# confluentinc/quickstart-streaming-agents

Measured on AMD Instinct MI355X. Metric: lab1_price_match_agent_decisions_per_sec, higher is better.
Workload: dtype bf16; 1 GPU; model=llama3-8b, global_batch=192, seq_len=2048, agent_loop=model_driven_grammar, parallelism=dp1

## Files before the change

quickstart_streaming_agents_amd/models/llama.py:

```python

from __future__ import annotations

import os
from dataclasses import dataclass

import torch
import torch.nn.functional as F

from ..ops import dispatch as D
from .kv_cache import PagedKVCache

PREFILL_V1 = os.environ.get("QSA_PREFILL_V1") == "1"
DECODE_V1 = os.environ.get("QSA_DECODE_V1") == "1"
PREFILL_TILE_ROWS = 32


@dataclass
class LlamaConfig:
    name: str = "llama3-8b"
    vocab_size: int = 128_256
    hidden: int = 4096
    n_layers: int = 32
    n_q_heads: int = 32
    n_kv_heads: int = 8
# ... 123 lines not shown
                if want(self.lm_head.shape):
                    self.lm_head_f = D.pack_weight_frag(self.lm_head)

    def _ffn_weights(self, w, rows, cols) -> dict:
        c = self.cfg
        wgu_full = w(2 * c.ffn, c.hidden)
        wgu = torch.cat([rows(wgu_full[:c.ffn], self.tp_size),
                         rows(wgu_full[c.ffn:], self.tp_size)],
                        dim=0).contiguous()
        wdown = cols(w(c.hidden, c.ffn, std=0.02 / (2 * c.n_layers) ** 0.5),
                     self.tp_size)
        return {"wgu": wgu, "wdown": wdown}

    def new_kv_cache(self, n_pages: int) -> PagedKVCache:
        return PagedKVCache(self.cfg.n_layers, self.n_kv, self.cfg.d_head,
                            n_pages, self.device, self.dtype)

    def _linear(self, x: torch.Tensor, w: torch.Tensor,
                wf: torch.Tensor | None = None,
                wf8: tuple | None = None) -> torch.Tensor:
        n, k = w.shape
        M = x.shape[0]
        if x.is_cuda and wf8 is not None:
            if M <= 32:
                return D.skinny_linear_fp8(x, wf8[0], wf8[1], n, k)
            import os as _os
            if _os.environ.get("QSA_FP8_BATCH") == "1" and M <= 256 \
                    and n % 64 == 0 and n <= 32768:
                wgs = n // 64
                splitk = 1 if wgs >= 256 else (2 if wgs >= 128 else 4)
                if k % (64 * splitk) == 0:
                    return D.gemm_fp8_batch(x, wf8[0], wf8[1], n, k,
                                            splitk)
        if x.is_cuda and M <= 32 and wf is not None and \
                n * k <= 6144 * 4096:
            return D.skinny_linear(x, wf, n, k)
        return F.linear(x, w)

    def _tp_all_reduce(self, t: torch.Tensor) -> torch.Tensor:
        if self.tp_size > 1:
            import torch.distributed as dist
            dist.all_reduce(t, group=self.tp_group)
        return t

    def _split_qkv(self, qkv: torch.Tensor, n: int):
        c = self.cfg
        qd = self.n_q * c.d_head
# ... 216 lines not shown
```

quickstart_streaming_agents_amd/models/serve.py:

```python

from __future__ import annotations

import time
from dataclasses import dataclass, field

import torch

from .llama import LlamaModel


@dataclass
class Sequence:
    seq_id: int
    prompt: list[int]
    max_new_tokens: int
    cached_len: int = 0
    out_tokens: list[int] = field(default_factory=list)
    done: bool = False
    keep_alive: bool = False
    decision_allowed: list[int] | None = None
    branches: dict[int, list[int]] | None = None
    script: list[int] | None = None


@dataclass
class EngineStats:
    prefill_tokens: int = 0
    cached_prefix_tokens: int = 0
    decode_tokens: int = 0
    decode_steps: int = 0
    jump_forward_tokens: int = 0
    prefills: int = 0
    prefill_batches: int = 0
    wall_s: float = 0.0
    prefill_s: float = 0.0
    decode_s: float = 0.0


import os as _os
_TIMING = _os.environ.get("QSA_TIMING", "") == "1"
_TUNABLE_DONE = False


def _enable_tunableop() -> None:
    global _TUNABLE_DONE
    if _TUNABLE_DONE or _os.environ.get("QSA_NO_TUNABLEOP") == "1":
        return
    _TUNABLE_DONE = True
    try:
        path = _os.path.join(_os.path.dirname(_os.path.abspath(__file__)),
                             "..", "data", "tunableop_mi355x.csv")
        if _os.path.exists(path):
            t = torch.cuda.tunable
            t.enable(True)
            t.tuning_enable(False)
            t.read_file(path)
    except Exception:
        pass


class Engine:
    def __init__(self, model: LlamaModel, kv_pages: int | None = None,
                 max_batch: int = 256, max_seq_len: int = 4096,
                 eos_id: int | None = None, prefill_batch_tokens: int = 65536,
# ... 2 lines not shown
                 decision_temperature: float = 1.0):
        if torch.cuda.is_available():
            _enable_tunableop()
        self.model = model
        self.temperature = float(temperature)
        self.decision_temperature = float(decision_temperature)
        self.jump_forward = _os.environ.get(
            "QSA_NO_JUMP_FORWARD", "") != "1"
        self.max_batch = max_batch
        self.max_seq_len = max_seq_len
        self.eos_id = eos_id
        self.prefill_batch_tokens = prefill_batch_tokens
        if kv_pages is None:
            kv_pages = max_batch * ((max_seq_len + 63) // 64) + 64
        self.kv = model.new_kv_cache(kv_pages)
        self._next_id = 0
        self.pending: list[Sequence] = []
        self.running: list[Sequence] = []
        self.finished: list[Sequence] = []
        self.stats = EngineStats()
        self.use_graph = torch.cuda.is_available() and \
            torch.device(model.device).type == "cuda"
        self._graph = None
        self._graph_failed = False
        self._gbuf: dict = {}
        self._vocab_bias: torch.Tensor | None = None
        if valid_vocab is not None:
            lo, hi = valid_vocab
            bias = torch.full((model.cfg.vocab_size,), float("-inf"),
                              device=model.device, dtype=torch.float32)
            bias[lo:hi] = 0.0
            if self.eos_id is not None:
                bias[self.eos_id] = 0.0
            self._vocab_bias = bias

    def _sample(self, logits: torch.Tensor) -> torch.Tensor:
        if self._vocab_bias is not None:
            logits = logits.float() + self._vocab_bias
        if self.temperature <= 0.0:
            return torch.argmax(logits, dim=-1)
        u = torch.rand(logits.shape, device=logits.device,
                       dtype=torch.float32).clamp_min_(1e-20)
        gumbel = -torch.log(-torch.log(u).clamp_min_(1e-20))
        return torch.argmax(logits.float() + self.temperature * gumbel,
                            dim=-1)

    def _sample_first(self, logits: torch.Tensor,
                      admitted: list["Sequence"]) -> list[int]:
        free = self._sample(logits)
        rows = [i for i, s in enumerate(admitted) if s.decision_allowed]
        if not rows:
# ... 13 lines not shown
            u = torch.rand(sub.shape, device=sub.device).clamp_min_(1e-20)
            sub = sub / t + (-torch.log(-torch.log(u)))
        sub = sub.masked_fill(pad, float("-inf"))
        pick = idx.gather(1, torch.argmax(sub, 1, keepdim=True)).squeeze(1)
        out = free.tolist()
        for r, t in zip(rows, pick.tolist()):
            out[r] = int(t)
        return [int(t) for t in out]

    MAX_RUN = 512

    def _ensure_graph(self) -> bool:
        if self._graph is not None:
            return True
        if self._graph_failed:
            return False
        try:
            self._capture_graph()
            return True
        except Exception:
            self._graph_failed = True
            self.use_graph = False
            self._graph = None
            torch.cuda.synchronize()
            return False

    def _capture_graph(self) -> None:
        dev = self.model.device
        B = self.max_batch
        cap = (self.max_seq_len + 63) // 64
        gb = {
            "tokens": torch.zeros(B, dtype=torch.int64, device=dev),
            "block_table": torch.zeros(B, cap, dtype=torch.int32, device=dev),
            "seq_lens": torch.zeros(B, dtype=torch.int32, device=dev),
            "active": torch.zeros(B, dtype=torch.int32, device=dev),
            "ctr": torch.zeros(1, dtype=torch.int64, device=dev),
            "hist": torch.zeros(self.MAX_RUN, B, dtype=torch.int64, device=dev),
            "script": torch.zeros(B, self.MAX_RUN, dtype=torch.int64,
                                  device=dev),
            "script_mask": torch.zeros(B, self.MAX_RUN, dtype=torch.bool,
                                       device=dev),
        }

        def body():
            gb["seq_lens"].add_(gb["active"])
            positions = (gb["seq_lens"] - 1).clamp(min=0).int()
            logits = self.model.forward_decode(
                gb["tokens"], self.kv, gb["block_table"], gb["seq_lens"],
                positions)
            nxt = self._sample(logits)
            j = gb["ctr"].clamp(max=self.MAX_RUN - 1)
            forced = gb["script"].index_select(1, j).squeeze(1)
            fmask = gb["script_mask"].index_select(1, j).squeeze(1)
            nxt = torch.where(fmask, forced, nxt)
            gb["hist"].index_copy_(0, gb["ctr"], nxt.unsqueeze(0))
            gb["ctr"].add_(1)
            gb["tokens"].copy_(nxt)

        for _ in range(2):
            body()
        gb["ctr"].zero_()
        gb["seq_lens"].zero_()
        torch.cuda.synchronize()
        g = torch.cuda.CUDAGraph()
        with torch.cuda.graph(g):
            body()
        self._graph = g
        self._gbuf = gb

    def _decode_run_eager(self, batch: list[Sequence], run: int) -> None:
        for _ in range(run):
            live = [s for s in batch if not s.done]
            if not live:
                break
            for s in live:
                self.kv.extend(s.seq_id, len(s.prompt) + len(s.out_tokens))
            self._decode_step_eager(live)

    def _decode_step_eager(self, batch: list[Sequence]) -> None:
        dev = self.model.device
        tokens = torch.tensor([s.out_tokens[-1] for s in batch],
                              dtype=torch.int64, device=dev)
        positions = torch.tensor(
            [len(s.prompt) + len(s.out_tokens) - 1 for s in batch],
            dtype=torch.int32, device=dev)
        seq_ids = [s.seq_id for s in batch]
        bt = self.kv.block_table(seq_ids)
        sl = self.kv.seq_lens_tensor(seq_ids)
        logits = self.model.forward_decode(tokens, self.kv, bt, sl,
                                           positions)
        nxt = self._sample(logits).tolist()
        for s, tok in zip(batch, nxt):
            if s.script:
                si = len(s.out_tokens) - 1
                if si < len(s.script):
                    tok = s.script[si]
            s.out_tokens.append(int(tok))
            self._maybe_finish(s)
        self.stats.decode_tokens += len(batch)
        self.stats.decode_steps += 1

    def _decode_run_graph(self, batch: list[Sequence], run: int) -> None:
        if not self._ensure_graph():
            self._decode_run_eager(batch, run)
            return
        self._graph_run_begin(batch, run)
        self._graph_run_end(batch, run)

    def _graph_run_begin(self, batch: list[Sequence], run: int) -> None:
        gb = self._gbuf
        n = len(batch)
        dev = self.model.device
        for s in batch:
            self.kv.extend(s.seq_id, len(s.prompt) + len(s.out_tokens) + run)
            self.kv._seq_len[s.seq_id] = \
                len(s.prompt) + len(s.out_tokens) - 1
        seq_ids = [s.seq_id for s in batch]
        bt = self.kv.block_table(seq_ids)
        gb["block_table"][:n, :bt.shape[1]] = bt
        gb["seq_lens"][:n] = self.kv.seq_lens_tensor(seq_ids)
        gb["tokens"][:n] = torch.tensor([s.out_tokens[-1] for s in batch],
                                        dtype=torch.int64, device=dev)
        gb["active"][:n] = 1
# ... 3 lines not shown
        if any(s.script for s in batch):
            sc = torch.zeros(n, run, dtype=torch.int64)
            sm = torch.zeros(n, run, dtype=torch.bool)
            for i, s in enumerate(batch):
                if not s.script:
                    continue
                d = len(s.out_tokens)
                window = s.script[d - 1: d - 1 + run]
                if window:
                    sc[i, :len(window)] = torch.tensor(window,
                                                       dtype=torch.int64)
                    sm[i, :len(window)] = True
            gb["script"][:n, :run] = sc.to(dev)
            gb["script_mask"][:n, :run] = sm.to(dev)
            gb["script_mask"][:n, run:] = False
            if n < self.max_batch:
                gb["script_mask"][n:] = False
        else:
            gb["script_mask"].fill_(False)
        gb["ctr"].zero_()
        if _TIMING:
            torch.cuda.synchronize()
            self._t_graph0 = time.perf_counter()
        for _ in range(run):
            self._graph.replay()

    def _graph_run_end(self, batch: list[Sequence], run: int) -> None:
        gb = self._gbuf
        n = len(batch)
        if _TIMING:
            torch.cuda.synchronize()
            self.stats.decode_s += time.perf_counter() - self._t_graph0
        hist = gb["hist"][:run, :n].t().tolist()
        for s, toks in zip(batch, hist):
            new = [int(t) for t in toks]
            if self.eos_id is not None and self.eos_id in new:
                new = new[: new.index(self.eos_id) + 1]
            s.out_tokens.extend(new)
            self.kv._seq_len[s.seq_id] = len(s.prompt) + len(s.out_tokens)
            self._maybe_finish(s)
        self.stats.decode_tokens += n * run
        self.stats.decode_steps += run

    def submit(self, prompt_tokens: list[int], max_new_tokens: int,
               continue_from: Sequence | None = None,
               keep_alive: bool = False, constraint=None) -> Sequence:
        prompt = list(prompt_tokens[: self.max_seq_len - 1])
        decision_allowed = branches = None
        if constraint is not None:
            decision_allowed = list(constraint.decision_allowed)
            branches = dict(constraint.branches)
            max_new_tokens = max(max_new_tokens,
                                 constraint.max_script_len() + 1)
            max_new_tokens = min(max_new_tokens, self.MAX_RUN)
        max_new_tokens = max(1, min(max_new_tokens,
                                    self.max_seq_len - len(prompt)))
        if continue_from is not None and not continue_from.keep_alive:
            continue_from = None
        if continue_from is not None:
            shared = min(len(continue_from.prompt), len(prompt) - 1)
            if prompt[:shared] != continue_from.prompt[:shared]:
                shared = 0
            if shared > 0:
                seq = Sequence(continue_from.seq_id, prompt, max_new_tokens,
                               cached_len=shared, keep_alive=keep_alive,
# ... 232 lines not shown
```

quickstart_streaming_agents_amd/ops/dispatch.py:

```python

from __future__ import annotations

import torch

from . import ext


def _cuda(t: torch.Tensor) -> bool:
    return t.is_cuda



def rmsnorm(x: torch.Tensor, w: torch.Tensor, eps: float) -> torch.Tensor:
    if _cuda(x):
        return ext().rmsnorm(x, w, eps)
    xf = x.float()
    y = xf * torch.rsqrt(xf.pow(2).mean(-1, keepdim=True) + eps) * w.float()
    return y.to(x.dtype)


def rmsnorm_residual(x: torch.Tensor, res: torch.Tensor, w: torch.Tensor,
                     eps: float) -> torch.Tensor:
    if _cuda(x):
        return ext().rmsnorm_residual(x, res, w, eps)
# ... 175 lines not shown
                      k: int) -> torch.Tensor:
    q = qf.reshape(n // 16, k // 64, 16, 4, 2, 8) \
        .permute(0, 2, 1, 4, 3, 5).reshape(n, k)
    return q.view(torch.float8_e4m3fn).float() * scale[:, None].float()


def gemm_fp8_batch(x: torch.Tensor, qf: torch.Tensor,
                   scale: torch.Tensor, n: int, k: int,
                   splitk: int = 1) -> torch.Tensor:
    if x.is_cuda:
        return ext().gemm_fp8_batch(x, qf, scale, n, k, splitk)
    w = unpack_weight_fp8(qf, scale, n, k)
    return (x.float() @ w.T).to(x.dtype)


def skinny_linear_fp8(x: torch.Tensor, qf: torch.Tensor,
                      scale: torch.Tensor, n: int, k: int) -> torch.Tensor:
    if x.is_cuda:
        return ext().skinny_gemm_fp8(x, qf, scale, n, k)
    w = unpack_weight_fp8(qf, scale, n, k)
    return (x.float() @ w.T).to(x.dtype)



def topk_cosine(queries: torch.Tensor, docs: torch.Tensor, k: int):
    if _cuda(queries):
        return ext().topk_cosine(queries, docs, k)
    from .cpu_ref import topk_cosine_ref
    return topk_cosine_ref(queries, docs, k)


def window_agg(ts: torch.Tensor, key: torch.Tensor,
               value: torch.Tensor | None, t0: int, win_ms: int, nwin: int,
               nkeys: int):
    if _cuda(ts):
        return ext().window_agg(ts, key, value, t0, win_ms, nwin, nkeys)
    from .cpu_ref import window_agg_ref
    return window_agg_ref(ts, key, value, t0, win_ms, nwin, nkeys)



def hash_build(keys: torch.Tensor, ts: torch.Tensor):
    ts = ts.clamp(min=0, max=(1 << 40) - 1)
    if _cuda(keys):
        return tuple(ext().hash_build(keys, ts.contiguous()))
    table: dict = {}
# ... 17 lines not shown
```

quickstart_streaming_agents_amd/ops/hip/elementwise.hip:

```cpp
#include "common.h"

__global__ void __launch_bounds__(256)
qsa_rmsnorm_kernel(const unsigned short* __restrict__ x,
                   const unsigned short* __restrict__ w,
                   unsigned short* __restrict__ y,
                   unsigned short* __restrict__ res,
                   int H, float eps) {
  const long long row = blockIdx.x;
  const unsigned short* xr = x + row * H;
  unsigned short* yr = y + row * H;
  unsigned short* rr = res ? res + row * H : nullptr;
  __shared__ float scratch[8];

  uint4 buf[4];
  float ss = 0.f;
#pragma unroll
  for (int c = 0; c < 4; ++c) {
    const int i = (threadIdx.x + c * blockDim.x) * 8;
    if (i >= H) break;
    uint4 v = *reinterpret_cast<const uint4*>(xr + i);
    float acc = 0.f;
    unsigned int pk[4] = {v.x, v.y, v.z, v.w};
    if (rr) {
      uint4 rv = *reinterpret_cast<const uint4*>(rr + i);
// ... 273 lines not shown
    uint4 o4;
    unsigned int* oo = reinterpret_cast<unsigned int*>(&o4);
#pragma unroll
    for (int j = 0; j < 4; ++j) {
      float2 f = bf16x2_to_f32x2(vv[j]);
      const float a = (i + 2 * j < limit) ? __expf(f.x * scale - mx) * inv
                                          : 0.f;
      const float b = (i + 2 * j + 1 < limit)
                          ? __expf(f.y * scale - mx) * inv : 0.f;
      oo[j] = f32x2_to_bf16x2(a, b);
    }
    *reinterpret_cast<uint4*>(r + i) = o4;
  }
}

extern "C" void qsa_softmax_rows_bf16_launch(unsigned short* scores,
                                             long long rows, int cols,
                                             float scale,
                                             const int* row_limits,
                                             hipStream_t stream) {
  hipLaunchKernelGGL(qsa_softmax_rows_bf16_kernel, dim3((unsigned)rows),
                     dim3(256), 0, stream, scores, cols, scale, row_limits);
}
```

quickstart_streaming_agents_amd/ops/hip/ops.cpp:

```cpp
#include <hip/hip_runtime.h>
#include <torch/extension.h>
#include <ATen/hip/HIPContext.h>

#define CHK(x) TORCH_CHECK(x, #x)
#define CHK_DEV(t) TORCH_CHECK((t).is_cuda(), #t " must be on the GPU")
#define CHK_CONT(t) TORCH_CHECK((t).is_contiguous(), #t " must be contiguous")
#define CHK_BF16(t) TORCH_CHECK((t).scalar_type() == at::kBFloat16, #t " must be bf16")
#define CHK_F32(t) TORCH_CHECK((t).scalar_type() == at::kFloat, #t " must be f32")
#define CHK_I32(t) TORCH_CHECK((t).scalar_type() == at::kInt, #t " must be i32")

static inline const unsigned short* u16(const torch::Tensor& t) {
  return reinterpret_cast<const unsigned short*>(t.data_ptr());
}
static inline unsigned short* u16m(torch::Tensor& t) {
  return reinterpret_cast<unsigned short*>(t.data_ptr());
}
static inline hipStream_t cur_stream() {
  return at::hip::getCurrentHIPStream().stream();
}

extern "C" void qsa_rmsnorm_launch(const unsigned short*, const unsigned short*,
                                   unsigned short*, unsigned short*, long long,
                                   int, float, hipStream_t);
extern "C" void qsa_swiglu_launch(const unsigned short*, const unsigned short*,
// ... 44 lines not shown
                                          hipStream_t);
extern "C" void qsa_kv_scatter_launch(const unsigned short*,
                                      const unsigned short*, unsigned short*,
                                      unsigned short*, const int*, int, int,
                                      int, long long, hipStream_t);
extern "C" void qsa_skinny_gemm_launch(const unsigned short*,
                                       const unsigned short*, unsigned short*,
                                       int, int, long long, long long,
                                       hipStream_t);
extern "C" void qsa_skinny_gemm_probe_launch(const unsigned short*,
                                             const unsigned short*,
                                             unsigned short*, int, int,
                                             long long, long long, int, int,
                                             int, hipStream_t);
extern "C" void qsa_skinny_gemm_fp8_launch(const unsigned short*,
                                           const unsigned char*,
                                           const float*, unsigned short*,
                                           int, int, long long, long long,
                                           hipStream_t);
extern "C" void qsa_skinny_gemm_fp8_probe_launch(
    const unsigned short*, const unsigned char*, const float*,
    unsigned short*, int, int, long long, long long, int, int, int,
    hipStream_t);
extern "C" void qsa_gemm_fp8_batch_launch(const unsigned short*,
                                          const unsigned char*,
                                          const float*, unsigned short*,
                                          float*, int, int, long long,
                                          long long, int, hipStream_t);
extern "C" void qsa_hash_build_launch(const long long*, const long long*,
                                      unsigned long long*,
                                      unsigned long long*, int, unsigned int,
                                      hipStream_t);
extern "C" void qsa_hash_probe_launch(const long long*,
                                      const unsigned long long*,
                                      const unsigned long long*, int*, int,
                                      unsigned int, long long, hipStream_t);
extern "C" void qsa_topk_launch(const float*, const float*, float*, int*,
                                float*, int*, int, int, int, int, int,
                                hipStream_t);
extern "C" void qsa_window_agg_launch(const long long*, const int*,
                                      const float*, int*, float*, long long,
                                      long long, int, long long, int,
                                      hipStream_t);
void register_avro(pybind11::module_&);
extern "C" void qsa_anomaly_batch_launch(const float*, const int*, float*,
                                         float*, int*, int, int, int,
// ... 432 lines not shown
  TORCH_CHECK(keys.scalar_type() == torch::kInt64 && keys.is_contiguous(),
              "keys must be contiguous i64");
  const long long m = keys.numel();
  const long long cap = tkeys.numel();
  TORCH_CHECK((cap & (cap - 1)) == 0, "table capacity must be pow2");
  auto out = torch::empty({m}, keys.options().dtype(torch::kInt32));
  qsa_hash_probe_launch((const long long*)keys.data_ptr<int64_t>(),
                        (const unsigned long long*)tkeys.data_ptr<int64_t>(),
                        (const unsigned long long*)tpay.data_ptr<int64_t>(),
                        out.data_ptr<int>(), (int)m,
                        (unsigned int)(cap - 1), min_ts, cur_stream());
  return out;
}

torch::Tensor skinny_gemm_fp8(torch::Tensor a, torch::Tensor qf,
                              torch::Tensor scale, long N, long K) {
  CHK_DEV(a); CHK_BF16(a); CHK_CONT(qf);
  TORCH_CHECK(qf.scalar_type() == torch::kUInt8, "qf must be uint8 (fp8)");
  TORCH_CHECK(scale.scalar_type() == torch::kFloat32 && scale.is_cuda() &&
                  scale.is_contiguous() && scale.numel() == N,
              "scale must be f32 [N] on device");
  TORCH_CHECK(a.dim() == 2 && a.stride(1) == 1, "a rows must be contiguous");
  const int M = a.size(0);
  TORCH_CHECK(M >= 1 && M <= 32, "skinny_gemm_fp8: M in [1,32]");
  TORCH_CHECK(a.size(1) == K, "K mismatch");
  TORCH_CHECK(K % 256 == 0 && N % 16 == 0, "K%256==0, N%16==0");
  TORCH_CHECK(qf.numel() == (long long)N * K, "qf size");
  auto out = torch::empty({M, (long long)N}, a.options());
  qsa_skinny_gemm_fp8_launch(u16(a), qf.data_ptr<unsigned char>(),
                             scale.data_ptr<float>(), u16m(out), M, (int)N,
                             K, a.stride(0), cur_stream());
  return out;
}

torch::Tensor skinny_gemm_fp8_probe(torch::Tensor a, torch::Tensor qf,
                                    torch::Tensor scale, long N, long K,
                                    long waves, long tiles, long nt) {
  CHK_DEV(a); CHK_BF16(a); CHK_CONT(qf);
  const int M = a.size(0);
  auto out = torch::empty({M, (long long)N}, a.options());
  qsa_skinny_gemm_fp8_probe_launch(u16(a), qf.data_ptr<unsigned char>(),
                                   scale.data_ptr<float>(), u16m(out), M,
                                   (int)N, K, a.stride(0), (int)waves,
                                   (int)tiles, (int)nt, cur_stream());
  return out;
}

std::vector<torch::Tensor> topk_cosine(torch::Tensor queries,
                                       torch::Tensor docs, long k) {
  CHK_DEV(queries); CHK_CONT(queries); CHK_F32(queries); CHK_F32(docs);
  CHK_CONT(docs);
  const int Q = queries.size(0), D = queries.size(1), N = docs.size(0);
  TORCH_CHECK(docs.size(1) == D, "dim mismatch");
  TORCH_CHECK(k >= 1 && k <= 16, "k in [1,16]");
  const int nblk = std::max(1, (N + 2047) / 2048);
  auto opts_f = queries.options();
  auto opts_i = queries.options().dtype(at::kInt);
  auto cand_s = torch::empty({Q, nblk, k}, opts_f);
  auto cand_i = torch::empty({Q, nblk, k}, opts_i);
  auto out_s = torch::empty({Q, k}, opts_f);
  auto out_i = torch::empty({Q, k}, opts_i);
  qsa_topk_launch(queries.data_ptr<float>(), docs.data_ptr<float>(),
                  cand_s.data_ptr<float>(), cand_i.data_ptr<int>(),
                  out_s.data_ptr<float>(), out_i.data_ptr<int>(), Q, N, D,
                  (int)k, nblk, cur_stream());
  return {out_s, out_i};
}

// ... 55 lines not shown
        py::arg("vc"), py::arg("cos_t"), py::arg("sin_t"),
        py::arg("block_table"), py::arg("seq_lens"), py::arg("scale"),
        py::arg("waves_per_simd") = 2);
  m.def("kv_append", &kv_append, "append one step's k/v to the paged cache");
  m.def("paged_attn_prefill_tiled", &paged_attn_prefill_tiled,
        "varlen flash prefill attention, K/V pages shared through LDS");
  m.def("rope_kv_scatter", &rope_kv_scatter,
        "fused prefill rope + paged-cache scatter");
  m.def("rope_kv_append", &rope_kv_append,
        "fused decode rope + paged-cache append");
  m.def("kv_scatter", &kv_scatter, "scatter prefill k/v by slot ids");
  m.def("pack_weight_frag", &pack_weight_frag,
        "repack [N,K] bf16 into MFMA-fragment-major for skinny_gemm");
  m.def("skinny_gemm", &skinny_gemm,
        "decode-batch GEMM (M<=32) on the packed weight stream");
  m.def("skinny_gemm_probe", &skinny_gemm_probe,
        "ablation probe: waves/nt/variant sweep");
  m.def("skinny_gemm_fp8", &skinny_gemm_fp8,
        "fp8-weight decode GEMM (M<=32): half the weight stream");
  m.def("gemm_fp8_batch", &gemm_fp8_batch,
        "batched-M (<=256) fp8 weight-stream GEMM with optional split-K");
  m.def("skinny_gemm_fp8_probe", &skinny_gemm_fp8_probe,
        "fp8 ablation probe: waves/tiles/nt sweep");
  m.def("topk_cosine", &topk_cosine, "exact cosine top-k over the HBM index");
  m.def("hash_build", &hash_build,
        "build latest-per-key hash table from (keys, event ts)");
  m.def("hash_probe", &hash_probe,
        "probe the hash table with TTL cutoff -> row indices or -1");
  m.def("window_agg", &window_agg, "segmented (key, window) count/sum");
  m.def("anomaly_batch", &anomaly_batch, "batched AR+ridge anomaly scorer");
  register_avro(m);
}
```

quickstart_streaming_agents_amd/ops/hip/skinny_gemm_fp8.hip:

```cpp
#include "common.h"

using bf16x8 = __attribute__((ext_vector_type(8))) short;
using f32x2v = __attribute__((ext_vector_type(2))) float;
using f32x4 = __attribute__((ext_vector_type(4))) float;
using u32x4 = __attribute__((ext_vector_type(4))) unsigned int;

#define QSA_KCH8 256

__device__ __forceinline__ bf16x8 fp8x8_to_bf16x8(unsigned int a,
                                                  unsigned int b) {
  f32x2v f01 = __builtin_amdgcn_cvt_pk_f32_fp8(a, false);
  f32x2v f23 = __builtin_amdgcn_cvt_pk_f32_fp8(a, true);
  f32x2v f45 = __builtin_amdgcn_cvt_pk_f32_fp8(b, false);
  f32x2v f67 = __builtin_amdgcn_cvt_pk_f32_fp8(b, true);
  union { unsigned int u; float f; } u0, u1;
  unsigned int p[4];
  u0.f = f01.x; u1.f = f01.y;
  p[0] = __builtin_amdgcn_perm(u1.u, u0.u, 0x07060302u);
  u0.f = f23.x; u1.f = f23.y;
  p[1] = __builtin_amdgcn_perm(u1.u, u0.u, 0x07060302u);
  u0.f = f45.x; u1.f = f45.y;
  p[2] = __builtin_amdgcn_perm(u1.u, u0.u, 0x07060302u);
  u0.f = f67.x; u1.f = f67.y;
  p[3] = __builtin_amdgcn_perm(u1.u, u0.u, 0x07060302u);
  union { unsigned int u[4]; bf16x8 v; } out;
  out.u[0] = p[0]; out.u[1] = p[1]; out.u[2] = p[2]; out.u[3] = p[3];
  return out.v;
}

template <int WAVES, int TILES, bool NT>
__global__ void __launch_bounds__(WAVES * 64)
qsa_skinny_gemm_fp8_t(const unsigned short* __restrict__ A,
                      const u32x4* __restrict__ Qf,
                      const float* __restrict__ scale,
                      unsigned short* __restrict__ Cbf,
                      int M, int N, long long K, long long lda) {
  const int nt0 = blockIdx.x * TILES;
  const int wave = threadIdx.x >> 6;
  const int lane = threadIdx.x & 63;
  const long long kchunks = K / QSA_KCH8;

  f32x4 acc0[TILES], acc1[TILES];
#pragma unroll
  for (int t = 0; t < TILES; ++t) {
    acc0[t] = {0.f, 0.f, 0.f, 0.f};
    acc1[t] = {0.f, 0.f, 0.f, 0.f};
  }

  const int arow = lane & 15;
  const int akoff = (lane >> 4) * 8;
  const int r0 = min(arow, M - 1);
  const int r1 = min(16 + arow, M - 1);
  const unsigned short* a0base = A + (long long)r0 * lda + akoff;
  const unsigned short* a1base = A + (long long)r1 * lda + akoff;

  const u32x4* qbase[TILES];
#pragma unroll
  for (int t = 0; t < TILES; ++t)
    qbase[t] = Qf + ((long long)(nt0 + t) * (K >> 6)) * 64 +
               (long long)((lane & 15) * 4 + (lane >> 4));

  for (long long c = wave; c < kchunks; c += WAVES) {
    const long long k0 = c * QSA_KCH8;
#pragma unroll
    for (int s = 0; s < 4; ++s) {
      const long long kb = (k0 >> 6) + s;
      u32x4 q[TILES];
#pragma unroll
      for (int t = 0; t < TILES; ++t) {
        if (NT) {
          q[t] = __builtin_nontemporal_load(qbase[t] + kb * 64);
        } else {
          q[t] = *reinterpret_cast<const u32x4*>(
              __builtin_assume_aligned(qbase[t] + kb * 64, 16));
        }
      }
      const long long ak = k0 + s * 64;
      const bf16x8 a00 = *reinterpret_cast<const bf16x8*>(a0base + ak);
      const bf16x8 a10 = *reinterpret_cast<const bf16x8*>(a1base + ak);
      const bf16x8 a01 = *reinterpret_cast<const bf16x8*>(a0base + ak + 32);
      const bf16x8 a11 = *reinterpret_cast<const bf16x8*>(a1base + ak + 32);
#pragma unroll
      for (int t = 0; t < TILES; ++t) {
        const bf16x8 w0 = fp8x8_to_bf16x8(q[t].x, q[t].y);
        const bf16x8 w1 = fp8x8_to_bf16x8(q[t].z, q[t].w);
        acc0[t] =
            __builtin_amdgcn_mfma_f32_16x16x32_bf16(a00, w0, acc0[t], 0, 0, 0);
        acc1[t] =
            __builtin_amdgcn_mfma_f32_16x16x32_bf16(a10, w0, acc1[t], 0, 0, 0);
        acc0[t] =
            __builtin_amdgcn_mfma_f32_16x16x32_bf16(a01, w1, acc0[t], 0, 0, 0);
        acc1[t] =
            __builtin_amdgcn_mfma_f32_16x16x32_bf16(a11, w1, acc1[t], 0, 0, 0);
      }
    }
  }

  __shared__ float red[WAVES][64][8];
#pragma unroll
  for (int t = 0; t < TILES; ++t) {
    if (t > 0) __syncthreads();
#pragma unroll
    for (int r = 0; r < 4; ++r) {
      red[wave][lane][r] = acc0[t][r];
      red[wave][lane][4 + r] = acc1[t][r];
    }
    __syncthreads();
    if (wave == 0) {
      const int ncol = (nt0 + t) * 16 + (lane & 15);
      const int mrow = (lane >> 4) * 4;
      const float s = scale[ncol];
#pragma unroll
      for (int r = 0; r < 4; ++r) {
        float v0 = 0.f, v1 = 0.f;
#pragma unroll
        for (int wv = 0; wv < WAVES; ++wv) {
          v0 += red[wv][lane][r];
          v1 += red[wv][lane][4 + r];
        }
        const int m0 = mrow + r;
        if (m0 < M) Cbf[(long long)m0 * N + ncol] = f32_to_bf16(v0 * s);
        if (16 + m0 < M)
          Cbf[(long long)(16 + m0) * N + ncol] = f32_to_bf16(v1 * s);
      }
    }
  }
}

extern "C" void qsa_skinny_gemm_fp8_launch(
    const unsigned short* A, const unsigned char* Qf, const float* scale,
    unsigned short* Cbf, int M, int N, long long K, long long lda,
    hipStream_t stream) {
  const u32x4* Q = reinterpret_cast<const u32x4*>(Qf);
  if (N % 128 == 0 && N >= 65536) {
    hipLaunchKernelGGL((qsa_skinny_gemm_fp8_t<2, 8, false>), dim3(N / 128),
                       dim3(128), 0, stream, A, Q, scale, Cbf, M, N, K,
                       lda);
  } else if (N % 64 == 0 && N >= 16384) {
    hipLaunchKernelGGL((qsa_skinny_gemm_fp8_t<8, 4, false>), dim3(N / 64),
                       dim3(512), 0, stream, A, Q, scale, Cbf, M, N, K,
                       lda);
  } else if (N % 32 == 0 && N >= 6144 && K < 8192) {
    hipLaunchKernelGGL((qsa_skinny_gemm_fp8_t<8, 2, false>), dim3(N / 32),
                       dim3(512), 0, stream, A, Q, scale, Cbf, M, N, K,
                       lda);
  } else {
    hipLaunchKernelGGL((qsa_skinny_gemm_fp8_t<8, 1, false>), dim3(N / 16),
                       dim3(512), 0, stream, A, Q, scale, Cbf, M, N, K,
                       lda);
  }
}

extern "C" void qsa_skinny_gemm_fp8_probe_launch(
    const unsigned short* A, const unsigned char* Qf, const float* scale,
    unsigned short* Cbf, int M, int N, long long K, long long lda,
    int waves, int tiles, int nt, hipStream_t stream) {
#define QSA_CASE(W, T, NTB)                                               \
  if (waves == W && tiles == T && nt == (int)NTB) {                       \
    hipLaunchKernelGGL((qsa_skinny_gemm_fp8_t<W, T, NTB>),                \
                       dim3(N / (16 * T)), dim3(W * 64), 0, stream, A,    \
                       reinterpret_cast<const u32x4*>(Qf), scale, Cbf,    \
                       M, N, K, lda);                                     \
    return;                                                               \
  }
  QSA_CASE(8, 1, false) QSA_CASE(8, 1, true) QSA_CASE(8, 2, false)
  QSA_CASE(8, 4, false) QSA_CASE(8, 4, true) QSA_CASE(8, 8, false)
  QSA_CASE(16, 1, false) QSA_CASE(16, 2, false) QSA_CASE(16, 4, false)
  QSA_CASE(4, 4, false) QSA_CASE(4, 8, false) QSA_CASE(2, 8, false)
#undef QSA_CASE
}
```

Baseline: 54.81 decisions/s.

## Add decode graph ladder, fused greedy sampler, and 64-row skinny fp8 GEMM

Captures several CUDA graphs at batch rungs (16/32/64/max) sharing one memory pool, so decode replays run only as many rows as are live instead of the full max batch. Adds a fused HIP kernel that does the windowed argmax, script override, history/token write and counter increment in one launch, replacing several small torch ops. Also generalises the skinny fp8 GEMM to up to four 16-row M tiles and routes wo projections with up to 64 rows through it. The costs are more graph capture time, the ticket-based atomic counter update, and added register pressure in the MT=4 kernel.

```diff
diff --git a/quickstart_streaming_agents_amd/models/llama.py b/quickstart_streaming_agents_amd/models/llama.py
--- a/quickstart_streaming_agents_amd/models/llama.py
+++ b/quickstart_streaming_agents_amd/models/llama.py
@@ -169,7 +169,7 @@
         n, k = w.shape
         M = x.shape[0]
         if x.is_cuda and wf8 is not None:
-            if M <= 32:
+            if M <= 32 or M <= D.skinny_fp8_row_limit(n, k):
                 return D.skinny_linear_fp8(x, wf8[0], wf8[1], n, k)
             import os as _os
             if _os.environ.get("QSA_FP8_BATCH") == "1" and M <= 256 \
diff --git a/quickstart_streaming_agents_amd/models/serve.py b/quickstart_streaming_agents_amd/models/serve.py
--- a/quickstart_streaming_agents_amd/models/serve.py
+++ b/quickstart_streaming_agents_amd/models/serve.py
@@ -35,11 +35,28 @@
     wall_s: float = 0.0
     prefill_s: float = 0.0
     decode_s: float = 0.0
+    decode_steps_by_live: dict = field(default_factory=dict)
+    decode_steps_by_rung: dict = field(default_factory=dict)
 
 
 import os as _os
 _TIMING = _os.environ.get("QSA_TIMING", "") == "1"
 _TUNABLE_DONE = False
+DECODE_LADDER = _os.environ.get("QSA_DECODE_LADDER", "1") != "0"
+LADDER_CANDIDATES = (16, 32, 64)
+
+
+def ladder_rungs(max_batch: int, ladder: bool = True) -> tuple:
+    if not ladder:
+        return (max_batch,)
+    return tuple(c for c in LADDER_CANDIDATES if c < max_batch) + (max_batch,)
+
+
+def pick_rung(rungs: tuple, n: int) -> int:
+    for r in rungs:
+        if r >= n:
+            return r
+    raise ValueError(f"{n} live rows exceed the largest rung {rungs[-1]}")
 
 
 def _enable_tunableop() -> None:
@@ -88,11 +105,15 @@
         self.use_graph = torch.cuda.is_available() and \
             torch.device(model.device).type == "cuda"
         self._graph = None
+        self._graphs: dict = {}
+        self._rungs: tuple = ()
         self._graph_failed = False
         self._gbuf: dict = {}
         self._vocab_bias: torch.Tensor | None = None
+        self._valid_vocab = None
         if valid_vocab is not None:
             lo, hi = valid_vocab
+            self._valid_vocab = (int(lo), int(hi))
             bias = torch.full((model.cfg.vocab_size,), float("-inf"),
                               device=model.device, dtype=torch.float32)
             bias[lo:hi] = 0.0
@@ -152,10 +173,16 @@
             self._graph_failed = True
             self.use_graph = False
             self._graph = None
+            self._graphs = {}
             torch.cuda.synchronize()
             return False
 
+    def _fused_sampler(self, logits: torch.Tensor) -> bool:
+        return self.temperature <= 0.0 and self._valid_vocab is not None \
+            and logits.is_cuda and logits.dtype == torch.bfloat16
+
     def _capture_graph(self) -> None:
+        from ..ops import dispatch as D
         dev = self.model.device
         B = self.max_batch
         cap = (self.max_seq_len + 63) // 64
@@ -170,32 +197,49 @@
                                   device=dev),
             "script_mask": torch.zeros(B, self.MAX_RUN, dtype=torch.bool,
                                        device=dev),
+            "ticket": torch.zeros(1, dtype=torch.int32, device=dev),
         }
-
-        def body():
-            gb["seq_lens"].add_(gb["active"])
-            positions = (gb["seq_lens"] - 1).clamp(min=0).int()
+        eos = -1 if self.eos_id is None else int(self.eos_id)
+
+        def body(b: int):
+            tokens, seq_lens = gb["tokens"][:b], gb["seq_lens"][:b]
+            seq_lens.add_(gb["active"][:b])
             logits = self.model.forward_decode(
-                gb["tokens"], self.kv, gb["block_table"], gb["seq_lens"],
-                positions)
+                tokens, self.kv, gb["block_table"][:b], seq_lens, None)
+            if self._fused_sampler(logits):
+                lo, hi = self._valid_vocab
+                D.greedy_sample_step(
+                    logits, lo, hi, eos, gb["script"][:b],
+                    gb["script_mask"][:b], gb["ctr"], gb["hist"][:, :b],
+                    tokens, gb["ticket"])
+                return
             nxt = self._sample(logits)
             j = gb["ctr"].clamp(max=self.MAX_RUN - 1)
-            forced = gb["script"].index_select(1, j).squeeze(1)
-            fmask = gb["script_mask"].index_select(1, j).squeeze(1)
+            forced = gb["script"][:b].index_select(1, j).squeeze(1)
+            fmask = gb["script_mask"][:b].index_select(1, j).squeeze(1)
             nxt = torch.where(fmask, forced, nxt)
-            gb["hist"].index_copy_(0, gb["ctr"], nxt.unsqueeze(0))
+            gb["hist"][:, :b].index_copy_(0, gb["ctr"], nxt.unsqueeze(0))
             gb["ctr"].add_(1)
-            gb["tokens"].copy_(nxt)
-
-        for _ in range(2):
-            body()
-        gb["ctr"].zero_()
-        gb["seq_lens"].zero_()
-        torch.cuda.synchronize()
-        g = torch.cuda.CUDAGraph()
-        with torch.cuda.graph(g):
-            body()
-        self._graph = g
+            tokens.copy_(nxt)
+
+        rungs = ladder_rungs(B, DECODE_LADDER)
+        graphs: dict = {}
+        pool = None
+        for b in reversed(rungs):
+            for _ in range(2):
+                body(b)
+            gb["ctr"].zero_()
+            gb["seq_lens"].zero_()
+            torch.cuda.synchronize()
+            g = torch.cuda.CUDAGraph()
+            with torch.cuda.graph(g, pool=pool):
+                body(b)
+            if pool is None:
+                pool = g.pool()
+            graphs[b] = g
+        self._graphs = graphs
+        self._rungs = rungs
+        self._graph = graphs[B]
         self._gbuf = gb
 
     def _decode_run_eager(self, batch: list[Sequence], run: int) -> None:
@@ -229,6 +273,8 @@
             self._maybe_finish(s)
         self.stats.decode_tokens += len(batch)
         self.stats.decode_steps += 1
+        by_live = self.stats.decode_steps_by_live
+        by_live[len(batch)] = by_live.get(len(batch), 0) + 1
 
     def _decode_run_graph(self, batch: list[Sequence], run: int) -> None:
         if not self._ensure_graph():
@@ -278,8 +324,10 @@
         if _TIMING:
             torch.cuda.synchronize()
             self._t_graph0 = time.perf_counter()
+        self._rung = pick_rung(self._rungs, n)
+        g = self._graphs[self._rung]
         for _ in range(run):
-            self._graph.replay()
+            g.replay()
 
     def _graph_run_end(self, batch: list[Sequence], run: int) -> None:
         gb = self._gbuf
@@ -297,6 +345,10 @@
             self._maybe_finish(s)
         self.stats.decode_tokens += n * run
         self.stats.decode_steps += run
+        by_live = self.stats.decode_steps_by_live
+        by_live[n] = by_live.get(n, 0) + run
+        by_rung = self.stats.decode_steps_by_rung
+        by_rung[self._rung] = by_rung.get(self._rung, 0) + run
 
     def submit(self, prompt_tokens: list[int], max_new_tokens: int,
                continue_from: Sequence | None = None,
diff --git a/quickstart_streaming_agents_amd/ops/dispatch.py b/quickstart_streaming_agents_amd/ops/dispatch.py
--- a/quickstart_streaming_agents_amd/ops/dispatch.py
+++ b/quickstart_streaming_agents_amd/ops/dispatch.py
@@ -221,6 +221,58 @@
     return (x.float() @ w.T).to(x.dtype)
 
 
+SKINNY_FP8_WIDE_CLASSES: frozenset = frozenset({"wo"})
+
+
+def skinny_fp8_class(n: int, k: int) -> str:
+    if n % 128 == 0 and n >= 65536:
+        return "lm_head"
+    if n % 64 == 0 and n >= 16384:
+        return "wgu"
+    if n % 32 == 0 and n >= 6144 and k < 8192:
+        return "qkv"
+    return "wo" if k < 8192 else "wdown"
+
+
+def skinny_fp8_row_limit(n: int, k: int) -> int:
+    return 64 if skinny_fp8_class(n, k) in SKINNY_FP8_WIDE_CLASSES else 32
+
+
+
+def greedy_sample_step(logits: torch.Tensor, lo: int, hi: int, eos: int,
+                       script: torch.Tensor, script_mask: torch.Tensor,
+                       ctr: torch.Tensor, hist: torch.Tensor,
+                       tokens: torch.Tensor,
+                       ticket: torch.Tensor | None = None) -> None:
+    if logits.is_cuda:
+        ext().greedy_sample_step(logits, lo, hi, eos, script, script_mask,
+                                 ctr, hist, tokens, ticket)
+        return
+    B = logits.shape[0]
+    if B == 0:
+        return
+    win = logits[:, lo:hi].float()
+    if hi > lo:
+        bv, bi = win.max(dim=1)
+        bi = (win == bv[:, None]).int().argmax(dim=1) + lo
+    else:
+        bv = torch.full((B,), float("-inf"))
+        bi = torch.zeros(B, dtype=torch.int64)
+    if eos >= 0 and not lo <= eos < hi:
+        ev = logits[:, eos].float()
+        take = (ev > bv) | ((ev == bv) & (eos < bi))
+        bi = torch.where(take, torch.full_like(bi, eos), bi)
+        bv = torch.where(take, ev, bv)
+    bi = torch.where(bv == float("-inf"), torch.zeros_like(bi), bi)
+    c = int(ctr[0])
+    j = min(max(c, 0), script.shape[1] - 1)
+    tok = torch.where(script_mask[:B, j], script[:B, j], bi)
+    if 0 <= c < hist.shape[0]:
+        hist[c, :B] = tok
+    tokens[:B] = tok
+    ctr.add_(1)
+
+
 
 def topk_cosine(queries: torch.Tensor, docs: torch.Tensor, k: int):
     if _cuda(queries):
diff --git a/quickstart_streaming_agents_amd/ops/hip/elementwise.hip b/quickstart_streaming_agents_amd/ops/hip/elementwise.hip
--- a/quickstart_streaming_agents_amd/ops/hip/elementwise.hip
+++ b/quickstart_streaming_agents_amd/ops/hip/elementwise.hip
@@ -319,3 +319,83 @@
   hipLaunchKernelGGL(qsa_softmax_rows_bf16_kernel, dim3((unsigned)rows),
                      dim3(256), 0, stream, scores, cols, scale, row_limits);
 }
+
+__device__ __forceinline__ void qsa_argmax_take(float& bv, int& bi, float v,
+                                                int i) {
+  if (v > bv || (v == bv && i < bi)) { bv = v; bi = i; }
+}
+
+__global__ void __launch_bounds__(256)
+qsa_greedy_sample_kernel(const unsigned short* __restrict__ logits,
+                         long long V, int lo, int hi, int eos,
+                         const long long* __restrict__ script,
+                         const unsigned char* __restrict__ script_mask,
+                         int max_run,
+                         long long* __restrict__ ctr,
+                         long long* __restrict__ hist,
+                         long long hist_stride, int hist_rows,
+                         long long* __restrict__ tokens,
+                         unsigned int* __restrict__ ticket) {
+  const int row = blockIdx.x;
+  const unsigned short* r = logits + (long long)row * V;
+  const float ninf = -__builtin_inff();
+  float bv = ninf;
+  int bi = 0;
+
+  const int mis = (int)((reinterpret_cast<unsigned long long>(r + lo) >> 1) & 7);
+  const int body0 = min(hi, lo + ((8 - mis) & 7));
+  const int body1 = body0 + ((hi - body0) & ~7);
+  for (int i = lo + threadIdx.x; i < body0; i += blockDim.x)
+    qsa_argmax_take(bv, bi, bf16_to_f32(r[i]), i);
+  for (int i = body0 + threadIdx.x * 8; i < body1; i += blockDim.x * 8) {
+    const uint4 v4 = *reinterpret_cast<const uint4*>(r + i);
+    const unsigned int vv[4] = {v4.x, v4.y, v4.z, v4.w};
+#pragma unroll
+    for (int j = 0; j < 4; ++j) {
+      const float2 f = bf16x2_to_f32x2(vv[j]);
+      qsa_argmax_take(bv, bi, f.x, i + 2 * j);
+      qsa_argmax_take(bv, bi, f.y, i + 2 * j + 1);
+    }
+  }
+  for (int i = body1 + threadIdx.x; i < hi; i += blockDim.x)
+    qsa_argmax_take(bv, bi, bf16_to_f32(r[i]), i);
+  if (threadIdx.x == 0 && eos >= 0 && (eos < lo || eos >= hi))
+    qsa_argmax_take(bv, bi, bf16_to_f32(r[eos]), eos);
+
+#pragma unroll
+  for (int off = 32; off > 0; off >>= 1) {
+    const float ov = __shfl_xor(bv, off, QSA_WAVE);
+    const int oi = __shfl_xor(bi, off, QSA_WAVE);
+    qsa_argmax_take(bv, bi, ov, oi);
+  }
+  __shared__ float sv[4];
+  __shared__ int si[4];
+  const int lane = threadIdx.x & 63, wave = threadIdx.x >> 6;
+  if (lane == 0) { sv[wave] = bv; si[wave] = bi; }
+  __syncthreads();
+  if (threadIdx.x == 0) {
+    for (int w = 1; w < 4; ++w) qsa_argmax_take(bv, bi, sv[w], si[w]);
+    const long long c = ctr[0];
+    const long long j = c < (long long)max_run - 1 ? (c < 0 ? 0 : c)
+                                                   : (long long)max_run - 1;
+    const long long so = (long long)row * max_run + j;
+    const long long tok = script_mask[so] ? script[so] : (long long)bi;
+    if (c >= 0 && c < hist_rows) hist[c * hist_stride + row] = tok;
+    tokens[row] = tok;
+    __threadfence();
+    if (atomicAdd(ticket, 1u) == gridDim.x - 1) {
+      ctr[0] = c + 1;
+      *ticket = 0u;
+    }
+  }
+}
+
+extern "C" void qsa_greedy_sample_launch(
+    const unsigned short* logits, int B, long long V, int lo, int hi, int eos,
+    const long long* script, const unsigned char* script_mask, int max_run,
+    long long* ctr, long long* hist, long long hist_stride, int hist_rows,
+    long long* tokens, unsigned int* ticket, hipStream_t stream) {
+  hipLaunchKernelGGL(qsa_greedy_sample_kernel, dim3(B), dim3(256), 0, stream,
+                     logits, V, lo, hi, eos, script, script_mask, max_run,
+                     ctr, hist, hist_stride, hist_rows, tokens, ticket);
+}
diff --git a/quickstart_streaming_agents_amd/ops/hip/ops.cpp b/quickstart_streaming_agents_amd/ops/hip/ops.cpp
--- a/quickstart_streaming_agents_amd/ops/hip/ops.cpp
+++ b/quickstart_streaming_agents_amd/ops/hip/ops.cpp
@@ -90,6 +90,14 @@
     const unsigned short*, const unsigned char*, const float*,
     unsigned short*, int, int, long long, long long, int, int, int,
     hipStream_t);
+extern "C" int qsa_skinny_gemm_fp8_probe_mt_launch(
+    const unsigned short*, const unsigned char*, const float*,
+    unsigned short*, int, int, long long, long long, int, int, int,
+    hipStream_t);
+extern "C" void qsa_greedy_sample_launch(
+    const unsigned short*, int, long long, int, int, int, const long long*,
+    const unsigned char*, int, long long*, long long*, long long, int,
+    long long*, unsigned int*, hipStream_t);
 extern "C" void qsa_gemm_fp8_batch_launch(const unsigned short*,
                                           const unsigned char*,
                                           const float*, unsigned short*,
@@ -568,7 +576,7 @@
               "scale must be f32 [N] on device");
   TORCH_CHECK(a.dim() == 2 && a.stride(1) == 1, "a rows must be contiguous");
   const int M = a.size(0);
-  TORCH_CHECK(M >= 1 && M <= 32, "skinny_gemm_fp8: M in [1,32]");
+  TORCH_CHECK(M >= 1 && M <= 64, "skinny_gemm_fp8: M in [1,64]");
   TORCH_CHECK(a.size(1) == K, "K mismatch");
   TORCH_CHECK(K % 256 == 0 && N % 16 == 0, "K%256==0, N%16==0");
   TORCH_CHECK(qf.numel() == (long long)N * K, "qf size");
@@ -590,6 +598,66 @@
                                    (int)N, K, a.stride(0), (int)waves,
                                    (int)tiles, (int)nt, cur_stream());
   return out;
+}
+
+torch::Tensor skinny_gemm_fp8_probe_mt(torch::Tensor a, torch::Tensor qf,
+                                       torch::Tensor scale, long N, long K,
+                                       long waves, long tiles, long mt) {
+  CHK_DEV(a); CHK_BF16(a); CHK_CONT(qf); CHK_DEV(qf); CHK_DEV(scale);
+  TORCH_CHECK(a.dim() == 2 && a.stride(1) == 1, "a rows must be contiguous");
+  const int M = a.size(0);
+  TORCH_CHECK(mt >= 1 && M >= 1 && M <= 16 * mt, "M in [1, 16*mt]");
+  TORCH_CHECK(a.size(1) == K && K % 256 == 0 && tiles >= 1 &&
+                  N % (16 * tiles) == 0,
+              "K%256==0, N%(16*tiles)==0");
+  TORCH_CHECK(qf.numel() == (long long)N * K && scale.numel() == N,
+              "qf / scale size");
+  auto out = torch::empty({M, (long long)N}, a.options());
+  const int ok = qsa_skinny_gemm_fp8_probe_mt_launch(
+      u16(a), qf.data_ptr<unsigned char>(), scale.data_ptr<float>(),
+      u16m(out), M, (int)N, K, a.stride(0), (int)waves, (int)tiles, (int)mt,
+      cur_stream());
+  TORCH_CHECK(ok, "skinny_gemm_fp8_probe_mt: variant not instantiated");
+  return out;
+}
+
+void greedy_sample_step(torch::Tensor logits, long lo, long hi, long eos,
+                        torch::Tensor script, torch::Tensor script_mask,
+                        torch::Tensor ctr, torch::Tensor hist,
+                        torch::Tensor tokens, torch::Tensor ticket) {
+  CHK_DEV(logits); CHK_CONT(logits); CHK_BF16(logits);
+  CHK_DEV(script); CHK_CONT(script); CHK_DEV(script_mask);
+  CHK_CONT(script_mask); CHK_DEV(ctr); CHK_DEV(hist); CHK_DEV(tokens);
+  CHK_CONT(tokens); CHK_DEV(ticket);
+  TORCH_CHECK(logits.dim() == 2, "logits [B, V]");
+  const long long B = logits.size(0), V = logits.size(1);
+  TORCH_CHECK(0 <= lo && lo <= hi && hi <= V, "0 <= lo <= hi <= V");
+  TORCH_CHECK(eos < V, "eos < V");
+  TORCH_CHECK(script.scalar_type() == at::kLong && script.dim() == 2 &&
+                  script.size(0) >= B, "script i64 [>=B, max_run]");
+  TORCH_CHECK(script_mask.scalar_type() == at::kBool &&
+                  script_mask.sizes() == script.sizes(),
+              "script_mask bool, same shape as script");
+  TORCH_CHECK(script.size(1) >= 1, "max_run >= 1");
+  TORCH_CHECK(ctr.scalar_type() == at::kLong && ctr.numel() == 1, "ctr i64 [1]");
+  TORCH_CHECK(hist.scalar_type() == at::kLong && hist.dim() == 2 &&
+                  hist.size(1) >= B && hist.stride(1) == 1,
+              "hist i64 [rows, >=B], unit column stride");
+  TORCH_CHECK(tokens.scalar_type() == at::kLong && tokens.numel() >= B,
+              "tokens i64 [>=B]");
+  TORCH_CHECK(ticket.scalar_type() == at::kInt && ticket.numel() == 1,
+              "ticket i32 [1]");
+  if (B == 0) return;
+  qsa_greedy_sample_launch(
+      u16(logits), (int)B, V, (int)lo, (int)hi, eos < 0 ? -1 : (int)eos,
+      reinterpret_cast<const long long*>(script.data_ptr<int64_t>()),
+      reinterpret_cast<const unsigned char*>(script_mask.data_ptr<bool>()),
+      (int)script.size(1),
+      reinterpret_cast<long long*>(ctr.data_ptr<int64_t>()),
+      reinterpret_cast<long long*>(hist.data_ptr<int64_t>()), hist.stride(0),
+      (int)hist.size(0),
+      reinterpret_cast<long long*>(tokens.data_ptr<int64_t>()),
+      reinterpret_cast<unsigned int*>(ticket.data_ptr<int>()), cur_stream());
 }
 
 std::vector<torch::Tensor> topk_cosine(torch::Tensor queries,
@@ -691,6 +759,11 @@
         "batched-M (<=256) fp8 weight-stream GEMM with optional split-K");
   m.def("skinny_gemm_fp8_probe", &skinny_gemm_fp8_probe,
         "fp8 ablation probe: waves/tiles/nt sweep");
+  m.def("skinny_gemm_fp8_probe_mt", &skinny_gemm_fp8_probe_mt,
+        "fp8 skinny GEMM with explicit (waves, tiles, m-tiles) for sweeps");
+  m.def("greedy_sample_step", &greedy_sample_step,
+        "fused greedy sampling step: windowed argmax, script override, "
+        "history/token/counter update (in place)");
   m.def("topk_cosine", &topk_cosine, "exact cosine top-k over the HBM index");
   m.def("hash_build", &hash_build,
         "build latest-per-key hash table from (keys, event ts)");
diff --git a/quickstart_streaming_agents_amd/ops/hip/skinny_gemm_fp8.hip b/quickstart_streaming_agents_amd/ops/hip/skinny_gemm_fp8.hip
--- a/quickstart_streaming_agents_amd/ops/hip/skinny_gemm_fp8.hip
+++ b/quickstart_streaming_agents_amd/ops/hip/skinny_gemm_fp8.hip
@@ -28,7 +28,7 @@
   return out.v;
 }
 
-template <int WAVES, int TILES, bool NT>
+template <int WAVES, int TILES, bool NT, int MT = 2>
 __global__ void __launch_bounds__(WAVES * 64)
 qsa_skinny_gemm_fp8_t(const unsigned short* __restrict__ A,
                       const u32x4* __restrict__ Qf,
@@ -40,19 +40,19 @@
   const int lane = threadIdx.x & 63;
   const long long kchunks = K / QSA_KCH8;
 
-  f32x4 acc0[TILES], acc1[TILES];
-#pragma unroll
-  for (int t = 0; t < TILES; ++t) {
-    acc0[t] = {0.f, 0.f, 0.f, 0.f};
-    acc1[t] = {0.f, 0.f, 0.f, 0.f};
+  f32x4 acc[MT][TILES];
+#pragma unroll
+  for (int m = 0; m < MT; ++m) {
+#pragma unroll
+    for (int t = 0; t < TILES; ++t) acc[m][t] = {0.f, 0.f, 0.f, 0.f};
   }
 
   const int arow = lane & 15;
   const int akoff = (lane >> 4) * 8;
-  const int r0 = min(arow, M - 1);
-  const int r1 = min(16 + arow, M - 1);
-  const unsigned short* a0base = A + (long long)r0 * lda + akoff;
-  const unsigned short* a1base = A + (long long)r1 * lda + akoff;
+  const unsigned short* abase[MT];
+#pragma unroll
+  for (int m = 0; m < MT; ++m)
+    abase[m] = A + (long long)min(16 * m + arow, M - 1) * lda + akoff;
 
   const u32x4* qbase[TILES];
 #pragma unroll
@@ -76,34 +76,36 @@
         }
       }
       const long long ak = k0 + s * 64;
-      const bf16x8 a00 = *reinterpret_cast<const bf16x8*>(a0base + ak);
-      const bf16x8 a10 = *reinterpret_cast<const bf16x8*>(a1base + ak);
-      const bf16x8 a01 = *reinterpret_cast<const bf16x8*>(a0base + ak + 32);
-      const bf16x8 a11 = *reinterpret_cast<const bf16x8*>(a1base + ak + 32);
+      bf16x8 a0[MT], a1[MT];
+#pragma unroll
+      for (int m = 0; m < MT; ++m) {
+        a0[m] = *reinterpret_cast<const bf16x8*>(abase[m] + ak);
+        a1[m] = *reinterpret_cast<const bf16x8*>(abase[m] + ak + 32);
+      }
 #pragma unroll
       for (int t = 0; t < TILES; ++t) {
         const bf16x8 w0 = fp8x8_to_bf16x8(q[t].x, q[t].y);
         const bf16x8 w1 = fp8x8_to_bf16x8(q[t].z, q[t].w);
-        acc0[t] =
-            __builtin_amdgcn_mfma_f32_16x16x32_bf16(a00, w0, acc0[t], 0, 0, 0);
-        acc1[t] =
-            __builtin_amdgcn_mfma_f32_16x16x32_bf16(a10, w0, acc1[t], 0, 0, 0);
-        acc0[t] =
-            __builtin_amdgcn_mfma_f32_16x16x32_bf16(a01, w1, acc0[t], 0, 0, 0);
-        acc1[t] =
-            __builtin_amdgcn_mfma_f32_16x16x32_bf16(a11, w1, acc1[t], 0, 0, 0);
+#pragma unroll
+        for (int m = 0; m < MT; ++m)
+          acc[m][t] = __builtin_amdgcn_mfma_f32_16x16x32_bf16(
+              a0[m], w0, acc[m][t], 0, 0, 0);
+#pragma unroll
+        for (int m = 0; m < MT; ++m)
+          acc[m][t] = __builtin_amdgcn_mfma_f32_16x16x32_bf16(
+              a1[m], w1, acc[m][t], 0, 0, 0);
       }
     }
   }
 
-  __shared__ float red[WAVES][64][8];
+  __shared__ float red[WAVES][64][4 * MT];
 #pragma unroll
   for (int t = 0; t < TILES; ++t) {
     if (t > 0) __syncthreads();
 #pragma unroll
-    for (int r = 0; r < 4; ++r) {
-      red[wave][lane][r] = acc0[t][r];
-      red[wave][lane][4 + r] = acc1[t][r];
+    for (int m = 0; m < MT; ++m) {
+#pragma unroll
+      for (int r = 0; r < 4; ++r) red[wave][lane][4 * m + r] = acc[m][t][r];
     }
     __syncthreads();
     if (wave == 0) {
@@ -111,19 +113,41 @@
       const int mrow = (lane >> 4) * 4;
       const float s = scale[ncol];
 #pragma unroll
-      for (int r = 0; r < 4; ++r) {
-        float v0 = 0.f, v1 = 0.f;
-#pragma unroll
-        for (int wv = 0; wv < WAVES; ++wv) {
-          v0 += red[wv][lane][r];
-          v1 += red[wv][lane][4 + r];
+      for (int m = 0; m < MT; ++m) {
+#pragma unroll
+        for (int r = 0; r < 4; ++r) {
+          float v = 0.f;
+#pragma unroll
+          for (int wv = 0; wv < WAVES; ++wv) v += red[wv][lane][4 * m + r];
+          const int mo = 16 * m + mrow + r;
+          if (mo < M) Cbf[(long long)mo * N + ncol] = f32_to_bf16(v * s);
         }
-        const int m0 = mrow + r;
-        if (m0 < M) Cbf[(long long)m0 * N + ncol] = f32_to_bf16(v0 * s);
-        if (16 + m0 < M)
-          Cbf[(long long)(16 + m0) * N + ncol] = f32_to_bf16(v1 * s);
       }
     }
+  }
+}
+
+template <int MT>
+static void qsa_skinny_gemm_fp8_launch_mt(
+    const unsigned short* A, const u32x4* Q, const float* scale,
+    unsigned short* Cbf, int M, int N, long long K, long long lda,
+    hipStream_t stream) {
+  if (N % 128 == 0 && N >= 65536) {
+    hipLaunchKernelGGL((qsa_skinny_gemm_fp8_t<2, 8, false, MT>),
+                       dim3(N / 128), dim3(128), 0, stream, A, Q, scale,
+                       Cbf, M, N, K, lda);
+  } else if (N % 64 == 0 && N >= 16384) {
+    hipLaunchKernelGGL((qsa_skinny_gemm_fp8_t<8, 4, false, MT>),
+                       dim3(N / 64), dim3(512), 0, stream, A, Q, scale, Cbf,
+                       M, N, K, lda);
+  } else if (N % 32 == 0 && N >= 6144 && K < 8192) {
+    hipLaunchKernelGGL((qsa_skinny_gemm_fp8_t<8, 2, false, MT>),
+                       dim3(N / 32), dim3(512), 0, stream, A, Q, scale, Cbf,
+                       M, N, K, lda);
+  } else {
+    hipLaunchKernelGGL((qsa_skinny_gemm_fp8_t<8, 1, false, MT>),
+                       dim3(N / 16), dim3(512), 0, stream, A, Q, scale, Cbf,
+                       M, N, K, lda);
   }
 }
 
@@ -132,23 +156,10 @@
     unsigned short* Cbf, int M, int N, long long K, long long lda,
     hipStream_t stream) {
   const u32x4* Q = reinterpret_cast<const u32x4*>(Qf);
-  if (N % 128 == 0 && N >= 65536) {
-    hipLaunchKernelGGL((qsa_skinny_gemm_fp8_t<2, 8, false>), dim3(N / 128),
-                       dim3(128), 0, stream, A, Q, scale, Cbf, M, N, K,
-                       lda);
-  } else if (N % 64 == 0 && N >= 16384) {
-    hipLaunchKernelGGL((qsa_skinny_gemm_fp8_t<8, 4, false>), dim3(N / 64),
-                       dim3(512), 0, stream, A, Q, scale, Cbf, M, N, K,
-                       lda);
-  } else if (N % 32 == 0 && N >= 6144 && K < 8192) {
-    hipLaunchKernelGGL((qsa_skinny_gemm_fp8_t<8, 2, false>), dim3(N / 32),
-                       dim3(512), 0, stream, A, Q, scale, Cbf, M, N, K,
-                       lda);
-  } else {
-    hipLaunchKernelGGL((qsa_skinny_gemm_fp8_t<8, 1, false>), dim3(N / 16),
-                       dim3(512), 0, stream, A, Q, scale, Cbf, M, N, K,
-                       lda);
-  }
+  if (M <= 32)
+    qsa_skinny_gemm_fp8_launch_mt<2>(A, Q, scale, Cbf, M, N, K, lda, stream);
+  else
+    qsa_skinny_gemm_fp8_launch_mt<4>(A, Q, scale, Cbf, M, N, K, lda, stream);
 }
 
 extern "C" void qsa_skinny_gemm_fp8_probe_launch(
@@ -169,3 +180,21 @@
   QSA_CASE(4, 4, false) QSA_CASE(4, 8, false) QSA_CASE(2, 8, false)
 #undef QSA_CASE
 }
+
+extern "C" int qsa_skinny_gemm_fp8_probe_mt_launch(
+    const unsigned short* A, const unsigned char* Qf, const float* scale,
+    unsigned short* Cbf, int M, int N, long long K, long long lda,
+    int waves, int tiles, int mt, hipStream_t stream) {
+#define QSA_CASE(W, T, MTV)                                               \
+  if (waves == W && tiles == T && mt == MTV) {                            \
+    hipLaunchKernelGGL((qsa_skinny_gemm_fp8_t<W, T, false, MTV>),         \
+                       dim3(N / (16 * T)), dim3(W * 64), 0, stream, A,    \
+                       reinterpret_cast<const u32x4*>(Qf), scale, Cbf,    \
+                       M, N, K, lda);                                     \
+    return 1;                                                             \
+  }
+  QSA_CASE(2, 8, 2) QSA_CASE(8, 4, 2) QSA_CASE(8, 2, 2) QSA_CASE(8, 1, 2)
+  QSA_CASE(2, 8, 4) QSA_CASE(8, 4, 4) QSA_CASE(8, 2, 4) QSA_CASE(8, 1, 4)
+#undef QSA_CASE
+  return 0;
+}
```

Result: faster. 57.03 decisions/s (median of 6 runs) (+4.1%).
